# xiezheng-cs/PyTorch_Distributed_Template

Measured on AMD Instinct MI355X. Metric: images/sec (node) ResNet-18 DDP bs=1200/GPU at 1/2/4/8 MI355X, higher is better.
Workload: dtype bf16; 1 GPU; model=resnet18, global_batch=1200, parallelism=dp1, per_gpu_batch=1200, sync_bn=False, engine=native-hip, comm=none, grad_compress=none

## Files before the change

### csrc/bindings.cpp

```cpp
#include <torch/extension.h>
#include <ATen/hip/HIPContext.h>
#include <c10/hip/HIPCachingAllocator.h>
#include <c10/hip/HIPGuard.h>

#include <cstdio>
#include <algorithm>
#include <map>
#include <memory>
#include <mutex>
#include <optional>
#include <vector>
#include <stdexcept>
#include <string>

#include "common.h"
#include "dtypes.h"
#include "kernels/bn.h"
#include "kernels/bnact.h"
#include "kernels/conv1x1.h"
#include "kernels/conv_fwd.h"
#include "kernels/conv_l1.h"
#include "kernels/conv_wgrad.h"
#include "kernels/dwconv.h"
#include "kernels/fp32.h"
// ... 1446 lines not shown
  m.def("gconv_dgrad", &gconv_dgrad, py::arg("dy"), py::arg("wt"), py::arg("dx"), py::arg("N"), py::arg("P"),
        py::arg("Q"), py::arg("width"), py::arg("H"), py::arg("W"), py::arg("stride"), py::arg("phases"), py::arg("j"),
        py::arg("bm"), py::arg("bn"), py::arg("bn_y1") = py::none(), py::arg("bn_coef1") = py::none(),
        py::arg("bn_slots") = py::none());
  m.def("gconv_wgrad", &gconv_wgrad);
  m.def("gconv_slice", []() { return kGSlice; });
  m.def("gconv_wgrad_l1", &gconv_wgrad_l1);
  m.def("wgrad_reduce", &wgrad_reduce);
  m.def("wgrad_blocks_3x3c64", &wgrad_blocks_3x3c64);
  m.def("wgrad_3x3c64_supported", &wgrad_3x3c64_supported);
  m.def("conv_wgrad_3x3c64", &conv_wgrad_3x3c64, py::arg("x"), py::arg("dy"), py::arg("ws"), py::arg("N"), py::arg("H"),
        py::arg("W"), py::arg("pre_coef") = py::none());
  m.def("conv_fwd_pre", &conv_fwd_pre);
  m.def("conv1x1x", &conv1x1x);
  m.def("conv1x1x_supported", &conv1x1x_supported);
  m.def("conv_dgrad_persistent", &dgrad_persistent_kind);
  m.def("conv1x1x_mode", &conv1x1x_mode);
  m.def("conv1x1x_l1_mode", &conv1x1x_l1_mode);
  m.def("conv_fwd_pre_supported", &conv_fwd_pre_supported);
  m.def("bn_slot_sum", &bn_slot_sum);
  m.def("stat_slots", &stat_slots);
  m.def("conv_l1_set_pp", &pdt::conv_l1_set_pp, py::arg("mode"),
        "layer1 kernel choice: 1 = 8-wave ping-pong, 0 = 4-wave, -1 = PDT_CONV_L1_PP (default); returns the previous");
  m.def("conv32_set_halo", &pdt::conv32_set_halo, py::arg("on"),
        "fp32 3x3/s1 64-channel convolutions: 1 = halo kernel (default), 0 = per-tap "
        "restaging kernel; returns the previous setting");
  m.def("bn_finalize", &bn_finalize);
  m.def("bn_finalize_slots", &bn_finalize_slots);
  m.def("bn_bwd_finalize_slots", &bn_bwd_finalize_slots);
  m.def("bn_eval_coef", &bn_eval_coef);
  m.def("bn_apply", &bn_apply);
  m.def("bn_bwd_reduce_blocks", &bn_bwd_reduce_blocks);
  m.def("bn_bwd_reduce", &bn_bwd_reduce);
  m.def("bn_bwd_finalize", &bn_bwd_finalize);
  m.def("bn_bwd_apply", &bn_bwd_apply);
  m.def("bn_relu_maxpool", &bn_relu_maxpool, py::arg("y"), py::arg("coef"), py::arg("out"), py::arg("idx"),
        py::arg("N"), py::arg("H"), py::arg("W"), py::arg("C"), py::arg("pad") = 1);
  m.def("maxpool_bwd_relu", &maxpool_bwd_relu, py::arg("dp"), py::arg("idx"), py::arg("y"), py::arg("coef"),
        py::arg("dz"), py::arg("N"), py::arg("H"), py::arg("W"), py::arg("C"), py::arg("pad") = 1);
  m.def("stem_fwd", &stem_fwd);
  m.def("stem_fwd_supported", [](int64_t Hp, int64_t Wp, int64_t P, int64_t Q) {
    return pdt::stem_fwd_supported((int)Hp, (int)Wp, (int)P, (int)Q);
  });
  m.def("stem_pool_bwd_reduce", &stem_pool_bwd_reduce);
  m.def("stem_pool_bwd_reduce_out", &stem_pool_bwd_reduce_out);
  m.def("stem_pool_bwd_apply", &stem_pool_bwd_apply);
  m.def("bnact_stats", &bnact_stats, py::arg("x"), py::arg("slots"), py::arg("rows"), py::arg("C"));
// ... 66 lines not shown
```

### csrc/common.h

```cpp
#pragma once
#include <hip/hip_runtime.h>
#include <stdint.h>

#include "dtypes.h"

namespace pdt {

struct FastDiv {
  uint32_t mul;
  uint32_t shift;
};

inline FastDiv make_fastdiv(uint32_t d) {
  uint32_t s = 0;
  while ((2ull << s) <= d) ++s;
  if ((d & (d - 1)) == 0) return FastDiv{0u, s};
  const uint64_t m = ((1ull << (32 + s)) + d - 1) / d;
  return FastDiv{(uint32_t)m, s};
}

}

#ifdef __HIPCC__
#define PDT_DEVICE __device__ __forceinline__
// ... 113 lines not shown

PDT_DEVICE uint32_t fdiv(uint32_t x, FastDiv f) {
  return f.mul ? (__umulhi(x, f.mul) >> f.shift) : (x >> f.shift);
}

typedef __attribute__((address_space(3))) void lds_void_t;
constexpr uint32_t kOOB = 0x80000000u;

PDT_DEVICE __amdgpu_buffer_rsrc_t make_rsrc(const void* p, uint32_t bytes) {
  return __builtin_amdgcn_make_buffer_rsrc(const_cast<void*>(p), (short)0, (int)bytes, 0x00020000);
}

PDT_DEVICE void buf_lds16(__amdgpu_buffer_rsrc_t r, void* lds_dst, uint32_t voff) {
  __builtin_amdgcn_raw_ptr_buffer_load_lds(r, (lds_void_t*)lds_dst, 16, voff, 0, 0, 0);
}

PDT_DEVICE void buf_lds16_asm(__amdgpu_buffer_rsrc_t r, void* lds_dst, uint32_t voff) {
  const uint32_t m0v = (uint32_t)(uintptr_t)(lds_void_t*)lds_dst;
  asm volatile("s_mov_b32 m0, %0\n\tbuffer_load_dwordx4 %1, %2, 0 offen lds"
               :
               : "s"(m0v), "v"(voff), "s"(r)
               : "m0");
}

typedef uint32_t u32x4v __attribute__((ext_vector_type(4)));
typedef uint32_t u32x2v __attribute__((ext_vector_type(2)));
PDT_DEVICE u32x4v gload16_asm(const void* p) {
  u32x4v v;
  asm volatile("global_load_dwordx4 %0, %1, off" : "=v"(v) : "v"(p));
  return v;
}
PDT_DEVICE u32x2v gload8_asm(const void* p) {
  u32x2v v;
  asm volatile("global_load_dwordx2 %0, %1, off" : "=v"(v) : "v"(p));
  return v;
}

PDT_DEVICE int xcd_remap(int bid, int nwg) {
  const int q = nwg >> 3, r = nwg & 7;
  const int xcd = bid & 7, local = bid >> 3;
  return (xcd < r ? xcd * (q + 1) : r * (q + 1) + (xcd - r) * q) + local;
}

}
#endif

// ... 33 lines not shown
```

### csrc/kernels/conv_fwd.h

```cpp
#pragma once
#include <hip/hip_runtime.h>
#include <stdint.h>

#include "conv_geom.h"

namespace pdt {

constexpr int kStatSlots = 64;

void stat_rows_reduce_launch(const float* rows, int R, int CK, double* slots, hipStream_t s, int slots_ld = 0);


struct ConvFwdArgs : ConvGeom {
  const uint16_t* x;
  const uint16_t* w;
  uint16_t* y;
  const uint16_t* res;
  double* stats;
  int bnb;
  const uint16_t* bn_y1;
  const float* bn_coef1;
  const uint16_t* bn_y2;
  const float* bn_coef2;
  const uint8_t* bn_mask;
  int pair_skip;
  int res_phase = -1;
  int stage_out = 0;
  const float* pre_coef = nullptr;
  int ldy = 0, coef_ld = 0, stats_ld = 0;
  int nslice = 0;
  int64_t slice_wstride = 0;
  int srows_coff = 0;
};

void conv_fwd_launch(const ConvFwdArgs& a, int dtype, int bm, int bn, int bk, hipStream_t s);
int conv_fwd_m_tiles(int64_t M, int bm);

}
```

### csrc/kernels/conv_fwd.hip

```cpp
#include <cstdlib>

#include "../common.h"
#include "conv_fwd.h"
#include "conv_l1.h"

namespace pdt {

typedef __attribute__((address_space(3))) void lds_void;
typedef __attribute__((address_space(1))) void glb_void;

template <int CHUNKS>
PDT_DEVICE int swz(int row) { return (row >> 1) & (CHUNKS - 1); }

template <int DT, int EPI, int RES, int FN, int FM, int WN, int WM, int BN, int WAVES_M, int NW_, int SMEM = 0,
          bool PERM = false>
PDT_DEVICE void conv_epilogue(const ConvFwdArgs& a, f32x4_t (&acc)[FN][FM], int64_t m0, int n0, int tile_m, int wn,
                              int wm, int tid, int lane, char* smem) {
  using E = E16<DT>;
  const int fr = lane & 15, fq = lane >> 4;
  const int PQ = a.Pm * a.Qm;
  const FastDiv fd_pq{a.pq_mul, a.pq_shift}, fd_q{a.q_mul, a.q_shift};
  constexpr int KS = EPI == 0 ? 0 : (EPI == 4 ? 3 : 2);
  float sacc[FN][4][KS > 0 ? KS : 1];
#pragma unroll
  for (int i = 0; i < FN; ++i)
#pragma unroll
    for (int r = 0; r < 4; ++r)
#pragma unroll
      for (int k = 0; k < (KS > 0 ? KS : 1); ++k) sacc[i][r][k] = 0.f;

  constexpr int RED_BYTES = WAVES_M * BN * 3 * 4;
  float* cf = (float*)(smem + RED_BYTES);
  const int64_t LDY = a.ldy ? a.ldy : a.Kout;
  if constexpr (EPI >= 2) {
    const int CL = a.coef_ld ? a.coef_ld : a.Kout;
    for (int c = tid; c < BN; c += NW_ * 64) {
      const int n = n0 + c;
      cf[0 * BN + c] = a.bn_coef1[n];
      cf[1 * BN + c] = a.bn_coef1[CL + n];
      cf[2 * BN + c] = a.bn_coef1[2 * CL + n];
      cf[3 * BN + c] = a.bn_coef1[3 * CL + n];
      if constexpr (EPI == 4) {
        cf[4 * BN + c] = a.bn_coef2[2 * CL + n];
        cf[5 * BN + c] = a.bn_coef2[3 * CL + n];
      }
    }
    __syncthreads();
  }
  auto chan = [&](int i, int r) { return PERM ? (i >> 1) * 32 + 8 * fq + 4 * (i & 1) + r : i * 16 + 4 * fq + r; };
  static_assert(!PERM || FN % 2 == 0, "PERM pairs fragments");
  auto coef4 = [&](int q, int i) { return *(const float4*)(cf + q * BN + wn * WN + chan(i, 0)); };

  constexpr bool LY1 = EPI >= 2, LY2 = EPI == 4, LM = EPI == 3 || EPI == 4;
  static_assert(!LM || WN % 64 == 0, "bitmask epilogue needs 64-channel wave columns");
  constexpr int MW = LM ? WN / 64 : 1;
  constexpr int PER_J = FN * (2 * (RES != 0) + 2 * LY1 + 2 * LY2) + (LM ? 2 * MW : 0);
  constexpr int BUDGET = (FN * FM * 4 >= 128 ? 64 : 96) - (KS > 2 ? FN * 4 * (KS - 2) * 2 : 0);
  constexpr int JC = PER_J == 0 ? FM
                     : (8 * PER_J <= BUDGET && FM % 8 == 0) ? 8
                     : (4 * PER_J <= BUDGET && FM % 4 == 0) ? 4
                     : (2 * PER_J <= BUDGET && FM % 2 == 0) ? 2 : 1;
  static_assert(FM % JC == 0, "epilogue chunking");
  constexpr int BM_T = WAVES_M * WM;
  constexpr int SPITCH = BN * 2 + 16;
  constexpr int STG_OFF = 16384;
  constexpr bool FULL = SMEM >= STG_OFF + BM_T * SPITCH;
  constexpr bool PERGRP = !FULL && WAVES_M > 1 && EPI != 2 && SMEM >= STG_OFF + WM * SPITCH;
  constexpr bool CAN_STAGE = FULL || PERGRP;
  static_assert(!CAN_STAGE || RED_BYTES + 6 * BN * 4 <= STG_OFF, "epilogue LDS regions overlap");
  const bool stage = CAN_STAGE && a.stage_out;
  char* stg = smem + STG_OFF;
  const int srow0 = FULL ? wm * WM : 0;
  constexpr bool RC = RES == 2;
  const bool res_on = !RC || (int)blockIdx.y == a.res_phase;
  auto copy_rows = [&](int g) {
    constexpr int CPR = BN / 8;
    constexpr int SROWS = FULL ? BM_T : WM;
    for (int q = tid; q < SROWS * CPR; q += NW_ * 64) {
      const int row = q / CPR, ch = q - row * CPR;
      const int64_t m = m0 + (FULL ? 0 : g * WM) + row;
      if (m < a.M) {
        const int mm = (int)m;
        const int nimg = (int)fdiv((uint32_t)mm, fd_pq);
        const int rem = mm - nimg * PQ;
        const int i_ = (int)fdiv((uint32_t)rem, fd_q), j_ = rem - i_ * a.Qm;
        const int oh = i_ * a.ost_h + a.ooff_h, ow = j_ * a.ost_w + a.ooff_w;
        const int64_t ob = (((int64_t)nimg * a.OH + oh) * a.OW + ow) * LDY + n0 + ch * 8;
        *(uint4*)(a.y + ob) = *(const uint4*)(stg + row * SPITCH + ch * 16);
      }
    }
  };
  if constexpr (PERGRP) {
    if (stage)
      for (int g = 0; g < wm; ++g) {
        __syncthreads();
        copy_rows(g);
        __syncthreads();
      }
  }
#pragma unroll
  for (int jc = 0; jc < FM; jc += JC) {
    int64_t obase[JC];
    uint32_t rbase[RC ? JC : 1];
    bool valid[JC];
#pragma unroll
    for (int jj = 0; jj < JC; ++jj) {
      const int64_t m = m0 + wm * WM + (jc + jj) * 16 + fr;
      valid[jj] = m < a.M;
      const int mm = valid[jj] ? (int)m : 0;
      const int nimg = (int)fdiv((uint32_t)mm, fd_pq);
      const int rem = mm - nimg * PQ;
      const int i_ = (int)fdiv((uint32_t)rem, fd_q), j_ = rem - i_ * a.Qm;
      const int oh = i_ * a.ost_h + a.ooff_h, ow = j_ * a.ost_w + a.ooff_w;
      obase[jj] = (((int64_t)nimg * a.OH + oh) * a.OW + ow) * LDY;
      if constexpr (RC) rbase[jj] = (uint32_t)mm * (uint32_t)LDY;
    }
    uint2 p_res[RES ? JC : 1][RES ? FN : 1], p_y1[LY1 ? JC : 1][LY1 ? FN : 1], p_y2[LY2 ? JC : 1][LY2 ? FN : 1];
    uint64_t p_m[LM ? JC : 1][MW];
#pragma unroll
    for (int jj = 0; jj < JC; ++jj) {
      if constexpr (PERM) {
#pragma unroll
        for (int i = 0; i < FN; i += 2) {
          const int64_t o = obase[jj] + n0 + wn * WN + chan(i, 0);
          auto split = [&](uint2 (&dst)[FN], const uint4 v) {
            dst[i] = make_uint2(v.x, v.y);
            dst[i + 1] = make_uint2(v.z, v.w);
          };
          if constexpr (RES == 1) split(p_res[jj], *(const uint4*)(a.res + o));
          if constexpr (RC) split(p_res[jj], *(const uint4*)(a.res + rbase[jj] + (uint32_t)(n0 + wn * WN + chan(i, 0))));
          if constexpr (LY1) split(p_y1[jj], *(const uint4*)(a.bn_y1 + o));
          if constexpr (LY2) split(p_y2[jj], *(const uint4*)(a.bn_y2 + o));
        }
      } else {
#pragma unroll
        for (int i = 0; i < FN; ++i) {
          const int64_t o = obase[jj] + n0 + wn * WN + i * 16 + 4 * fq;
          if constexpr (RES == 1) p_res[jj][i] = *(const uint2*)(a.res + o);
          if constexpr (RC) p_res[jj][i] = *(const uint2*)(a.res + rbase[jj] + (uint32_t)(n0 + wn * WN + i * 16 + 4 * fq));
          if constexpr (LY1) p_y1[jj][i] = *(const uint2*)(a.bn_y1 + o);
          if constexpr (LY2) p_y2[jj][i] = *(const uint2*)(a.bn_y2 + o);
        }
      }
      if constexpr (LM) {
#pragma unroll
        for (int g = 0; g < MW; ++g)
          p_m[jj][g] = *(const uint64_t*)(a.bn_mask + ((obase[jj] + n0 + wn * WN + g * 64) >> 3));
      }
    }
#pragma unroll
    for (int jj = 0; jj < JC; ++jj) {
      if (!valid[jj]) continue;
      const int j = jc + jj;
      uint2 held = make_uint2(0u, 0u);
#pragma unroll
      for (int i = 0; i < FN; ++i) {
        const int n = n0 + wn * WN + chan(i, 0);
        const int64_t o = obase[jj] + n;
        float v[4] = {acc[i][j][0], acc[i][j][1], acc[i][j][2], acc[i][j][3]};
        if constexpr (RES) {
          uint2 rr = p_res[jj][i];
          if constexpr (RC) {
            rr.x = res_on ? rr.x : 0u;
            rr.y = res_on ? rr.y : 0u;
          }
          v[0] += E::to_f((uint16_t)(rr.x & 0xffff));
          v[1] += E::to_f((uint16_t)(rr.x >> 16));
          v[2] += E::to_f((uint16_t)(rr.y & 0xffff));
          v[3] += E::to_f((uint16_t)(rr.y >> 16));
        }
        float y1[4], y2[4];
        if constexpr (LY1) {
          const uint2 q1 = p_y1[jj][i];
          y1[0] = E::to_f((uint16_t)(q1.x & 0xffff)); y1[1] = E::to_f((uint16_t)(q1.x >> 16));
          y1[2] = E::to_f((uint16_t)(q1.y & 0xffff)); y1[3] = E::to_f((uint16_t)(q1.y >> 16));
          if constexpr (EPI == 2) {
            const float4 sc = coef4(0, i), sh = coef4(1, i);
            if (!(y1[0] * sc.x + sh.x > 0.f)) v[0] = 0.f;
            if (!(y1[1] * sc.y + sh.y > 0.f)) v[1] = 0.f;
            if (!(y1[2] * sc.z + sh.z > 0.f)) v[2] = 0.f;
            if (!(y1[3] * sc.w + sh.w > 0.f)) v[3] = 0.f;
          } else {
            const uint32_t mb = (uint32_t)(p_m[jj][chan(i, 0) >> 6] >> (chan(i, 0) & 63));
            if (!(mb & 1u)) v[0] = 0.f;
            if (!(mb & 2u)) v[1] = 0.f;
            if (!(mb & 4u)) v[2] = 0.f;
            if (!(mb & 8u)) v[3] = 0.f;
          }
        }
        if constexpr (LY2) {
          const uint2 q2 = p_y2[jj][i];
          y2[0] = E::to_f((uint16_t)(q2.x & 0xffff)); y2[1] = E::to_f((uint16_t)(q2.x >> 16));
          y2[2] = E::to_f((uint16_t)(q2.y & 0xffff)); y2[3] = E::to_f((uint16_t)(q2.y >> 16));
        }
        uint2 packed;
        packed.x = E::pack2(v[0], v[1]);
        packed.y = E::pack2(v[2], v[3]);
        const uint16_t ov[4] = {(uint16_t)packed.x, (uint16_t)(packed.x >> 16), (uint16_t)packed.y,
                                (uint16_t)(packed.y >> 16)};
        if (CAN_STAGE && stage) {
          if constexpr (PERM) {
            if (i & 1)
              *(uint4*)(stg + (srow0 + j * 16 + fr) * SPITCH + (wn * WN + chan(i, 0) - 4) * 2) =
                  make_uint4(held.x, held.y, packed.x, packed.y);
            else
              held = packed;
          } else {
            *(uint2*)(stg + (srow0 + j * 16 + fr) * SPITCH + (wn * WN + chan(i, 0)) * 2) = packed;
          }
        } else if constexpr (PERM) {
          if (i & 1)
            *(uint4*)(a.y + o - 4) = make_uint4(held.x, held.y, packed.x, packed.y);
          else
            held = packed;
        } else {
          *(uint2*)(a.y + o) = packed;
        }
        if constexpr (EPI == 1) {
#pragma unroll
          for (int r = 0; r < 4; ++r) {
            const float q = E::to_f(ov[r]);
            sacc[i][r][0] += q;
            sacc[i][r][1] += q * q;
          }
        } else if constexpr (EPI >= 2) {
          const float4 mu = coef4(2, i), is = coef4(3, i);
          const float m1[4] = {mu.x, mu.y, mu.z, mu.w}, i1[4] = {is.x, is.y, is.z, is.w};
#pragma unroll
          for (int r = 0; r < 4; ++r) {
            const float dz = E::to_f(ov[r]);
            sacc[i][r][0] += dz;
            sacc[i][r][1] += dz * (y1[r] - m1[r]) * i1[r];
          }
          if constexpr (EPI == 4) {
            const float4 mu2 = coef4(4, i), is2 = coef4(5, i);
            const float m2[4] = {mu2.x, mu2.y, mu2.z, mu2.w}, i2[4] = {is2.x, is2.y, is2.z, is2.w};
#pragma unroll
            for (int r = 0; r < 4; ++r) sacc[i][r][2] += E::to_f(ov[r]) * (y2[r] - m2[r]) * i2[r];
          }
        }
      }
    }
  }

  if constexpr (CAN_STAGE) {
    if (stage) {
      if constexpr (PERGRP) {
        for (int g = wm; g < WAVES_M; ++g) {
          __syncthreads();
          copy_rows(g);
          __syncthreads();
        }
      } else {
        __syncthreads();
        copy_rows(0);
      }
    }
  }

  if constexpr (KS > 0) {
    constexpr int KO = EPI == 4 ? 4 : 2;
#pragma unroll
    for (int i = 0; i < FN; ++i)
#pragma unroll
      for (int r = 0; r < 4; ++r)
#pragma unroll
        for (int k = 0; k < KS; ++k) sacc[i][r][k] = row16_sum(sacc[i][r][k]);
    float* red = (float*)smem;
    __syncthreads();
    if (fr == 15) {
#pragma unroll
      for (int i = 0; i < FN; ++i)
#pragma unroll
        for (int r = 0; r < 4; ++r) {
          const int nl = wn * WN + chan(i, r);
#pragma unroll
          for (int k = 0; k < KS; ++k) red[(wm * BN + nl) * KS + k] = sacc[i][r][k];
        }
// ... 9 lines not shown
        for (int k = 0; k < KS; ++k) t[k] += red[(w * BN + tid) * KS + k];
      const int64_t row = (a.nphase > 0 ? (int64_t)blockIdx.y * a.srows_pp : 0) + tile_m;
      const int64_t sld = a.nslice > 1 ? (int64_t)a.nslice * a.Kout : a.Kout;
      float* dst = a.srows + (row * sld + a.srows_coff + n0 + tid) * KO;
      if constexpr (EPI == 4)
        *(float4*)dst = make_float4(t[0], t[1], t[0], t[2]);
      else
        *(float2*)dst = make_float2(t[0], t[1]);
    }
  }
}

template <int EPI, int BN_>
PDT_DEVICE void zero_stat_row(const ConvFwdArgs& a, int nthreads) {
  if constexpr (EPI != 0) {
    constexpr int KO = EPI == 4 ? 4 : 2;
    const int tm = (int)blockIdx.x / a.n_tiles, tn = (int)blockIdx.x - tm * a.n_tiles;
    const int64_t sld = a.nslice > 1 ? (int64_t)a.nslice * a.Kout : a.Kout;
    float* dst = a.srows + (((int64_t)blockIdx.y * a.srows_pp + tm) * sld + a.srows_coff) * KO + (int64_t)tn * BN_ * KO;
    for (int i = threadIdx.x; i < BN_ * KO; i += nthreads) dst[i] = 0.f;
  }
}

template <int DT, int BM, int BN, int BK, int WAVES_N, int EPI, int RES, int STAGES, int NW>
__global__ __launch_bounds__(NW * 64, (STAGES * (BN + BM) * BK * 2 <= 81920 || NW == 8) ? 2 : 1)
void conv_fwd_kernel(ConvFwdArgs args) {
  ConvFwdArgs a = args;
  const uint16_t* wbase = args.w;
  if (args.nslice > 1) {
    const int sl = blockIdx.z;
    a.x += (int64_t)sl * a.Kout;
    a.y += (int64_t)sl * a.Kout;
    wbase += (int64_t)sl * args.slice_wstride;
    a.w = wbase;
    if (a.bn_y1 != nullptr) a.bn_y1 += (int64_t)sl * a.Kout;
    if (a.bn_coef1 != nullptr) a.bn_coef1 += sl * a.Kout;
    a.srows_coff = sl * a.Kout;
  }
  if (args.nphase > 0 && !select_phase(a, args, wbase, blockIdx.y)) {
    zero_stat_row<EPI, BN>(a, NW * 64);
    return;
  }
  using E = E16<DT>;
  typedef typename E::vec8 vec8;
  constexpr int WAVES_M = NW / WAVES_N;
  constexpr int WN = BN / WAVES_N;
  constexpr int WM = BM / WAVES_M;
// ... 146 lines not shown
        asm volatile("s_waitcnt vmcnt(0)" ::: "memory");
    };
    static_assert(S <= 4, "wait_ahead covers at most two stages in flight");
    if (ksteps > 0) {
#pragma unroll
      for (int p = 0; p < S - 1; ++p)
        if (p < ksteps) stage_load(p);
      int buf = 0;
      for (int ks = 0; ks < ksteps; ++ks) {
        const int ahead = min(S - 2, ksteps - 1 - ks);
        wait_ahead(ahead);
        __builtin_amdgcn_s_barrier();
        if (ks + S - 1 < ksteps) stage_load(buf == 0 ? S - 1 : buf - 1);
        __builtin_amdgcn_s_setprio(1);
        compute_stage(smem + buf * STAGE);
        __builtin_amdgcn_s_setprio(0);
        buf = buf == S - 1 ? 0 : buf + 1;
      }
      asm volatile("s_waitcnt lgkmcnt(0)" ::: "memory");
      __builtin_amdgcn_s_barrier();
    }
  }

  conv_epilogue<DT, EPI, RES, FN, FM, WN, WM, BN, WAVES_M, NW, STAGES * STAGE, PERM>(a, acc, m0, n0, tile_m, wn, wm, tid,
                                                                             lane, smem);
}

template <int N>
PDT_DEVICE void vm_wait() {
  static_assert(N >= 0 && N < 64, "vmcnt range");
  __builtin_amdgcn_s_waitcnt((N & 0xF) | ((N >> 4) << 14) | (0x7 << 4) | (0xF << 8));
}

template <int DT, int BM, int BN, int EPI, int RES, bool PP_STAGE = (EPI != 2)>
__global__ __launch_bounds__(512) void conv_pp_kernel(ConvFwdArgs args) {
  ConvFwdArgs a = args;
  if (args.nphase > 0 && !select_phase(a, args, args.w, blockIdx.y)) {
    zero_stat_row<EPI, BN>(a, 512);
    return;
  }
  using E = E16<DT>;
  typedef typename E::vec8 vec8;
  constexpr int NW = 8, WN = 64, WM = 128;
  constexpr int WAVES_N = BN / WN, WAVES_M = NW / WAVES_N;
  static_assert(WAVES_N * WAVES_M == NW && WAVES_M * WM == BM, "pp tile geometry");
  constexpr int FN = 4, FM = 8;
  constexpr int ROWB = 128;
  constexpr int XH = (BM / 2) * ROWB;
  constexpr int WH = (BN / 2) * ROWB;
  constexpr int NX = XH / 1024 / NW;
  constexpr int NWI = WH / 1024 / NW;
  static_assert(NX * 1024 * NW == XH && NWI * 1024 * NW == WH, "pp DMA split");
  constexpr int BUF = 2 * XH + 2 * WH;
  constexpr int OX0 = 0, OX1 = XH, OW0 = 2 * XH, OW1 = 2 * XH + WH;
  __shared__ __attribute__((aligned(1024))) char smem[2 * BUF];

  const int tid = threadIdx.x;
  const int lane = tid & 63;
  const int wave = __builtin_amdgcn_readfirstlane(tid >> 6);
  const int grp = wave >> 2;
  const int wn = wave % WAVES_N, wm = wave / WAVES_N;

  const int nwg = a.m_tiles * a.n_tiles;
  const int bid = xcd_remap(blockIdx.x, nwg);
  const int tile_m = bid / a.n_tiles, tile_n = bid % a.n_tiles;
  const int64_t m0 = (int64_t)tile_m * BM;
  const int n0 = tile_n * BN;

  const int PQ = a.Pm * a.Qm;
  const FastDiv fd_pq{a.pq_mul, a.pq_shift}, fd_q{a.q_mul, a.q_shift};
  const int TU = a.T * a.U;
  const int csteps = a.C >> 6;
  const int ksteps = TU * csteps;

  const __amdgpu_buffer_rsrc_t rx = make_rsrc(a.x, (uint32_t)a.N * a.H * a.W * a.cs * 2u);
  const __amdgpu_buffer_rsrc_t rw = make_rsrc(a.w, (uint32_t)a.Kout * TU * a.C * 2u);

  const int lrow = lane >> 3, pchunk = lane & 7;
// ... 114 lines not shown
    for (int ks = 0; ks < ksteps; ++ks) {
      const char* cb = smem + (ks & 1) * BUF;
      char* nb = smem + ((ks + 1) & 1) * BUF;
      const bool more = ks + 1 < ksteps;
      if (more) advance();
      if (more) { dma_x(nb, 0); vm_wait<2 * NX>(); } else { vm_wait<NX>(); }
      read_x(cb + OX0);
      read_w(w0r, cb + OW0);
      compute(w0r, 0, 0);
      if (more) { dma_w(nb, 0); vm_wait<NX + NWI>(); } else { vm_wait<0>(); }
      read_w(w1r, cb + OW1);
      compute(w1r, 0, 1);
      if (more) dma_w(nb, 1);
      read_x(cb + OX1);
      compute(w1r, 1, 1);
      if (more) { dma_x(nb, 1); vm_wait<NWI + NX>(); }
      compute(w0r, 1, 0);
    }
    if (grp == 0) __builtin_amdgcn_s_barrier();
    asm volatile("s_waitcnt vmcnt(0) lgkmcnt(0)" ::: "memory");
    __builtin_amdgcn_s_barrier();
  }

  conv_epilogue<DT, EPI, RES, FN, FM, WN, WM, BN, WAVES_M, NW, PP_STAGE ? 2 * BUF : 0, true>(a, acc, m0, n0, tile_m, wn,
                                                                                        wm, tid, lane, smem);
}

template <int DT, int BM, int BN>
static void launch_pp(const ConvFwdArgs& args, int gx, hipStream_t s) {
  ConvFwdArgs a = args;
  a.stage_out = 0;
  if (a.nslice > 1)
    pdt_hip_fail("conv_pp: slice-batched (grouped) launches run on the generic kernel", hipErrorInvalidValue, __FILE__,
                 __LINE__);
  dim3 grid(gx, a.nphase > 0 ? a.nphase : 1), block(512);
  const int rs = a.res == nullptr ? 0 : (a.res_phase >= 0 && a.nphase > 0 ? 2 : 1);
  const int epi = a.bnb ? a.bnb + 1 : (a.stats != nullptr ? 1 : 0);
#define PDT_K(E_, R_) hipLaunchKernelGGL((conv_pp_kernel<DT, BM, BN, E_, R_>), grid, block, 0, s, a)
  if (epi == 0) {
    if (rs == 1) PDT_K(0, 1); else if (rs == 2) PDT_K(0, 2); else PDT_K(0, 0);
  } else if (epi == 1 && rs != 2) {
    if (rs) PDT_K(1, 1); else PDT_K(1, 0);
  } else if (epi == 2 && !rs) {
    PDT_K(2, 0);
  } else if (epi == 3 && rs) {
    if (rs == 2) PDT_K(3, 2); else PDT_K(3, 1);
  } else if (epi == 4 && rs) {
    if (rs == 2) PDT_K(4, 2); else PDT_K(4, 1);
  } else {
    pdt_hip_fail("conv_pp: unsupported epilogue variant", hipErrorInvalidValue, __FILE__, __LINE__);
  }
#undef PDT_K
}

template <int DT, int BM, int BN, int BK, int WAVES_N, int STAGES, int NW>
static void launch_cfg(const ConvFwdArgs& a, int gx, hipStream_t s) {
  dim3 grid(gx, a.nphase > 0 ? a.nphase : 1, a.nslice > 1 ? a.nslice : 1), block(NW * 64);
  const int rs = a.res == nullptr ? 0 : (a.res_phase >= 0 && a.nphase > 0 ? 2 : 1);
  const int epi = a.bnb ? a.bnb + 1 : (a.stats != nullptr ? 1 : 0);
#define PDT_K(E_, R_) hipLaunchKernelGGL((conv_fwd_kernel<DT, BM, BN, BK, WAVES_N, E_, R_, STAGES, NW>), grid, block, 0, s, a)
  if (epi == 0) {
    if (rs == 1) PDT_K(0, 1); else if (rs == 2) PDT_K(0, 2); else PDT_K(0, 0);
  } else if (epi == 1 && rs != 2) {
    if (rs) PDT_K(1, 1); else PDT_K(1, 0);
  } else if constexpr ((((BK == 64 && STAGES == 2) || (BK == 32 && STAGES == 3)) && (BN == 128 || BN == 64) &&
                        (BM * BN == 4096 * NW || (BM == 256 && BN == 128 && NW == 4))) ||
                       (BM == 256 && BN == 256)) {
    if (epi == 2 && !rs) PDT_K(2, 0);
    else if (epi == 3 && rs) { if (rs == 2) PDT_K(3, 2); else PDT_K(3, 1); }
    else if (epi == 4 && rs) { if (rs == 2) PDT_K(4, 2); else PDT_K(4, 1); }
    else pdt_hip_fail("conv_fwd: unsupported BN-backward epilogue variant", hipErrorInvalidValue, __FILE__, __LINE__);
  } else {
    pdt_hip_fail("conv_fwd: BN-backward epilogue needs a 128x128 or 256x64 tile", hipErrorInvalidValue,
                 __FILE__, __LINE__);
  }
#undef PDT_K
}

template <int DT>
static void launch_tile(const ConvFwdArgs& a, int gx, int bm, int bn, int bk, hipStream_t s);

template <int DT>
static void launch_dt(ConvFwdArgs a, int bm, int bn, int bk, hipStream_t s) {
  a.stage_out = 0;
  int gx = 0;
  const int srows = conv_geom_plan(a, bm, bn, &gx);
  if (gx == 0) return;
  const int KO = a.bnb == 3 ? 4 : 2;
  const int nsl = a.nslice > 1 ? a.nslice : 1;
  Scratch part(a.stats ? (size_t)srows * a.Kout * nsl * KO * sizeof(float) : 0, s);
  a.srows = part.as<float>();
  launch_tile<DT>(a, gx, bm, bn, bk, s);
  if (a.stats) stat_rows_reduce_launch(a.srows, srows, a.Kout * nsl * KO, a.stats, s, a.stats_ld);
}

template <int DT>
static void launch_tile(const ConvFwdArgs& a, int gx, int bm, int bn, int bk, hipStream_t s) {
#define PDT_CFGN(BM_, BN_, BK_, WN_, ST_, NW_)            \
  if (bm == BM_ && bn == BN_ && bk == BK_) {               \
    launch_cfg<DT, BM_, BN_, BK_, WN_, ST_, NW_>(a, gx, s); \
    return;                                                \
  }
#define PDT_CFG(BM_, BN_, BK_, WN_, ST_) PDT_CFGN(BM_, BN_, BK_, WN_, ST_, 4)
  {
    const bool dg = a.nphase > 0;
    const bool pp = bk == 64 && a.C % 64 == 0 && ((bm == 256 && bn == 256) || (bm == 512 && bn == 128));
    if (pp && dg)
// ... 89 lines not shown
```

Baseline: 62390 images/s.

## Stream BN-backward epilogue operands through a per-wave LDS ring via buffer-to-LDS loads

Adds a RING variant of the conv epilogue for the BN-backward dgrad cases (EPI 3/4 with residual). It prefetches the residual, y1, y2 and mask operands for several output chunks into a per-wave LDS ring using buffer_load...lds, and waits on those loads with explicit vmcnt values, so global loads overlap the epilogue math instead of stalling on register-held chunks. It also removes the unused stage_out path that staged output through LDS. The ring is on by default and can be toggled with an env var or a new binding. In exchange it enlarges LDS in the pp kernel and relies on hand-tuned waitcnt counts.

Measured after the change: 62960 images/s, median of 6. Within noise of the previous version (+0.9%).

```diff
diff --git a/csrc/bindings.cpp b/csrc/bindings.cpp
--- a/csrc/bindings.cpp
+++ b/csrc/bindings.cpp
@@ -1492,7 +1492,10 @@
   m.def("stat_slots", &stat_slots);
   m.def("conv_l1_set_pp", &pdt::conv_l1_set_pp, py::arg("mode"),
         "layer1 kernel choice: 1 = 8-wave ping-pong, 0 = 4-wave, -1 = PDT_CONV_L1_PP (default); returns the previous");
-  m.def("conv32_set_halo", &pdt::conv32_set_halo, py::arg("on"),
+  m.def("conv_set_epi_ring", &pdt::conv_set_epi_ring, py::arg("mode"),
+        "operand ring of the block-output BN-backward dgrad epilogues: 1 = on, 0 = register chunks, "
+        "-1 = PDT_EPI_RING (default: on); returns the previous");
+  m.def("conv32_set_halo",&pdt::conv32_set_halo, py::arg("on"),
         "fp32 3x3/s1 64-channel convolutions: 1 = halo kernel (default), 0 = per-tap "
         "restaging kernel; returns the previous setting");
   m.def("bn_finalize", &bn_finalize);
diff --git a/csrc/common.h b/csrc/common.h
--- a/csrc/common.h
+++ b/csrc/common.h
@@ -159,6 +159,16 @@
                : "s"(m0v), "v"(voff), "s"(r)
                : "m0");
 }
+PDT_DEVICE void buf_lds4_lo32_asm(__amdgpu_buffer_rsrc_t r, void* lds_dst, uint32_t voff) {
+  const uint32_t m0v = (uint32_t)(uintptr_t)(lds_void_t*)lds_dst;
+  uint32_t hi;
+  asm volatile(
+      "s_mov_b32 m0, %1\n\ts_mov_b32 %0, exec_hi\n\ts_mov_b32 exec_hi, 0\n\t"
+      "buffer_load_dword %2, %3, 0 offen lds\n\ts_mov_b32 exec_hi, %0"
+      : "=&s"(hi)
+      : "s"(m0v), "v"(voff), "s"(r)
+      : "m0");
+}
 
 typedef uint32_t u32x4v __attribute__((ext_vector_type(4)));
 typedef uint32_t u32x2v __attribute__((ext_vector_type(2)));
diff --git a/csrc/kernels/conv_fwd.h b/csrc/kernels/conv_fwd.h
--- a/csrc/kernels/conv_fwd.h
+++ b/csrc/kernels/conv_fwd.h
@@ -25,7 +25,6 @@
   const uint8_t* bn_mask;
   int pair_skip;
   int res_phase = -1;
-  int stage_out = 0;
   const float* pre_coef = nullptr;
   int ldy = 0, coef_ld = 0, stats_ld = 0;
   int nslice = 0;
@@ -35,5 +34,6 @@
 
 void conv_fwd_launch(const ConvFwdArgs& a, int dtype, int bm, int bn, int bk, hipStream_t s);
 int conv_fwd_m_tiles(int64_t M, int bm);
+int conv_set_epi_ring(int mode);
 
 }
diff --git a/csrc/kernels/conv_fwd.hip b/csrc/kernels/conv_fwd.hip
--- a/csrc/kernels/conv_fwd.hip
+++ b/csrc/kernels/conv_fwd.hip
@@ -1,4 +1,6 @@
 #include <cstdlib>
+#include <type_traits>
+#include <utility>
 
 #include "../common.h"
 #include "conv_fwd.h"
@@ -12,8 +14,23 @@
 template <int CHUNKS>
 PDT_DEVICE int swz(int row) { return (row >> 1) & (CHUNKS - 1); }
 
+template <class F, int... Is>
+PDT_DEVICE void static_for_impl(F&& f, std::integer_sequence<int, Is...>) {
+  (f(std::integral_constant<int, Is>{}), ...);
+}
+template <int N, class F>
+PDT_DEVICE void static_for(F&& f) {
+  static_for_impl(f, std::make_integer_sequence<int, N>{});
+}
+
+template <int N>
+PDT_DEVICE void epi_vm_wait() {
+  static_assert(N >= 0 && N < 64, "vmcnt range");
+  asm volatile("s_waitcnt vmcnt(%0)" ::"n"(N) : "memory");
+}
+
 template <int DT, int EPI, int RES, int FN, int FM, int WN, int WM, int BN, int WAVES_M, int NW_, int SMEM = 0,
-          bool PERM = false>
+          bool PERM = false, bool RING = false>
 PDT_DEVICE void conv_epilogue(const ConvFwdArgs& a, f32x4_t (&acc)[FN][FM], int64_t m0, int n0, int tile_m, int wn,
                               int wm, int tid, int lane, char* smem) {
   using E = E16<DT>;
@@ -32,7 +49,7 @@
   constexpr int RED_BYTES = WAVES_M * BN * 3 * 4;
   float* cf = (float*)(smem + RED_BYTES);
   const int64_t LDY = a.ldy ? a.ldy : a.Kout;
-  if constexpr (EPI >= 2) {
+  auto stage_coefs = [&]() __attribute__((always_inline)) {
     const int CL = a.coef_ld ? a.coef_ld : a.Kout;
     for (int c = tid; c < BN; c += NW_ * 64) {
       const int n = n0 + c;
@@ -46,7 +63,8 @@
       }
     }
     __syncthreads();
-  }
+  };
+  if constexpr (EPI >= 2 && !RING) stage_coefs();
   auto chan = [&](int i, int r) { return PERM ? (i >> 1) * 32 + 8 * fq + 4 * (i & 1) + r : i * 16 + 4 * fq + r; };
   static_assert(!PERM || FN % 2 == 0, "PERM pairs fragments");
   auto coef4 = [&](int q, int i) { return *(const float4*)(cf + q * BN + wn * WN + chan(i, 0)); };
@@ -61,199 +79,236 @@
                      : (4 * PER_J <= BUDGET && FM % 4 == 0) ? 4
                      : (2 * PER_J <= BUDGET && FM % 2 == 0) ? 2 : 1;
   static_assert(FM % JC == 0, "epilogue chunking");
-  constexpr int BM_T = WAVES_M * WM;
-  constexpr int SPITCH = BN * 2 + 16;
-  constexpr int STG_OFF = 16384;
-  constexpr bool FULL = SMEM >= STG_OFF + BM_T * SPITCH;
-  constexpr bool PERGRP = !FULL && WAVES_M > 1 && EPI != 2 && SMEM >= STG_OFF + WM * SPITCH;
-  constexpr bool CAN_STAGE = FULL || PERGRP;
-  static_assert(!CAN_STAGE || RED_BYTES + 6 * BN * 4 <= STG_OFF, "epilogue LDS regions overlap");
-  const bool stage = CAN_STAGE && a.stage_out;
-  char* stg = smem + STG_OFF;
-  const int srow0 = FULL ? wm * WM : 0;
   constexpr bool RC = RES == 2;
   const bool res_on = !RC || (int)blockIdx.y == a.res_phase;
-  auto copy_rows = [&](int g) {
-    constexpr int CPR = BN / 8;
-    constexpr int SROWS = FULL ? BM_T : WM;
-    for (int q = tid; q < SROWS * CPR; q += NW_ * 64) {
-      const int row = q / CPR, ch = q - row * CPR;
-      const int64_t m = m0 + (FULL ? 0 : g * WM) + row;
-      if (m < a.M) {
-        const int mm = (int)m;
-        const int nimg = (int)fdiv((uint32_t)mm, fd_pq);
-        const int rem = mm - nimg * PQ;
-        const int i_ = (int)fdiv((uint32_t)rem, fd_q), j_ = rem - i_ * a.Qm;
-        const int oh = i_ * a.ost_h + a.ooff_h, ow = j_ * a.ost_w + a.ooff_w;
-        const int64_t ob = (((int64_t)nimg * a.OH + oh) * a.OW + ow) * LDY + n0 + ch * 8;
-        *(uint4*)(a.y + ob) = *(const uint4*)(stg + row * SPITCH + ch * 16);
-      }
-    }
-  };
-  if constexpr (PERGRP) {
-    if (stage)
-      for (int g = 0; g < wm; ++g) {
-        __syncthreads();
-        copy_rows(g);
-        __syncthreads();
-      }
-  }
-#pragma unroll
-  for (int jc = 0; jc < FM; jc += JC) {
-    int64_t obase[JC];
-    uint32_t rbase[RC ? JC : 1];
-    bool valid[JC];
-#pragma unroll
-    for (int jj = 0; jj < JC; ++jj) {
-      const int64_t m = m0 + wm * WM + (jc + jj) * 16 + fr;
-      valid[jj] = m < a.M;
-      const int mm = valid[jj] ? (int)m : 0;
-      const int nimg = (int)fdiv((uint32_t)mm, fd_pq);
-      const int rem = mm - nimg * PQ;
-      const int i_ = (int)fdiv((uint32_t)rem, fd_q), j_ = rem - i_ * a.Qm;
-      const int oh = i_ * a.ost_h + a.ooff_h, ow = j_ * a.ost_w + a.ooff_w;
-      obase[jj] = (((int64_t)nimg * a.OH + oh) * a.OW + ow) * LDY;
-      if constexpr (RC) rbase[jj] = (uint32_t)mm * (uint32_t)LDY;
-    }
-    uint2 p_res[RES ? JC : 1][RES ? FN : 1], p_y1[LY1 ? JC : 1][LY1 ? FN : 1], p_y2[LY2 ? JC : 1][LY2 ? FN : 1];
-    uint64_t p_m[LM ? JC : 1][MW];
-#pragma unroll
-    for (int jj = 0; jj < JC; ++jj) {
+  auto pixel = [&](int j, bool& ok, int64_t& ob, uint32_t& rb) __attribute__((always_inline)) {
+    const int64_t m = m0 + wm * WM + j * 16 + fr;
+    ok = m < a.M;
+    const int mm = ok ? (int)m : 0;
+    const int nimg = (int)fdiv((uint32_t)mm, fd_pq);
+    const int rem = mm - nimg * PQ;
+    const int i_ = (int)fdiv((uint32_t)rem, fd_q), j_ = rem - i_ * a.Qm;
+    const int oh = i_ * a.ost_h + a.ooff_h, ow = j_ * a.ost_w + a.ooff_w;
+    ob = (((int64_t)nimg * a.OH + oh) * a.OW + ow) * LDY;
+    rb = (uint32_t)mm * (uint32_t)LDY;
+  };
+  auto emit = [&](int j, int64_t ob, const uint2 (&pr)[RES ? FN : 1], const uint2 (&py1)[LY1 ? FN : 1],
+                  const uint2 (&py2)[LY2 ? FN : 1], const uint64_t (&pm)[MW]) __attribute__((always_inline)) {
+    uint2 held = make_uint2(0u, 0u);
+#pragma unroll
+    for (int i = 0; i < FN; ++i) {
+      const int n = n0 + wn * WN + chan(i, 0);
+      const int64_t o = ob + n;
+      float v[4] = {acc[i][j][0], acc[i][j][1], acc[i][j][2], acc[i][j][3]};
+      if constexpr (RES) {
+        uint2 rr = pr[i];
+        if constexpr (RC) {
+          rr.x = res_on ? rr.x : 0u;
+          rr.y = res_on ? rr.y : 0u;
+        }
+        v[0] += E::to_f((uint16_t)(rr.x & 0xffff));
+        v[1] += E::to_f((uint16_t)(rr.x >> 16));
+        v[2] += E::to_f((uint16_t)(rr.y & 0xffff));
+        v[3] += E::to_f((uint16_t)(rr.y >> 16));
+      }
+      float y1[4], y2[4];
+      if constexpr (LY1) {
+        const uint2 q1 = py1[i];
+        y1[0] = E::to_f((uint16_t)(q1.x & 0xffff)); y1[1] = E::to_f((uint16_t)(q1.x >> 16));
+        y1[2] = E::to_f((uint16_t)(q1.y & 0xffff)); y1[3] = E::to_f((uint16_t)(q1.y >> 16));
+        if constexpr (EPI == 2) {
+          const float4 sc = coef4(0, i), sh = coef4(1, i);
+          if (!(y1[0] * sc.x + sh.x > 0.f)) v[0] = 0.f;
+          if (!(y1[1] * sc.y + sh.y > 0.f)) v[1] = 0.f;
+          if (!(y1[2] * sc.z + sh.z > 0.f)) v[2] = 0.f;
+          if (!(y1[3] * sc.w + sh.w > 0.f)) v[3] = 0.f;
+        } else {
+          const uint32_t mb = (uint32_t)(pm[chan(i, 0) >> 6] >> (chan(i, 0) & 63));
+          if (!(mb & 1u)) v[0] = 0.f;
+          if (!(mb & 2u)) v[1] = 0.f;
+          if (!(mb & 4u)) v[2] = 0.f;
+          if (!(mb & 8u)) v[3] = 0.f;
+        }
+      }
+      if constexpr (LY2) {
+        const uint2 q2 = py2[i];
+        y2[0] = E::to_f((uint16_t)(q2.x & 0xffff)); y2[1] = E::to_f((uint16_t)(q2.x >> 16));
+        y2[2] = E::to_f((uint16_t)(q2.y & 0xffff)); y2[3] = E::to_f((uint16_t)(q2.y >> 16));
+      }
+      uint2 packed;
+      packed.x = E::pack2(v[0], v[1]);
+      packed.y = E::pack2(v[2], v[3]);
+      const uint16_t ov[4] = {(uint16_t)packed.x, (uint16_t)(packed.x >> 16), (uint16_t)packed.y,
+                              (uint16_t)(packed.y >> 16)};
       if constexpr (PERM) {
-#pragma unroll
-        for (int i = 0; i < FN; i += 2) {
-          const int64_t o = obase[jj] + n0 + wn * WN + chan(i, 0);
-          auto split = [&](uint2 (&dst)[FN], const uint4 v) {
-            dst[i] = make_uint2(v.x, v.y);
-            dst[i + 1] = make_uint2(v.z, v.w);
+        if (i & 1)
+          *(uint4*)(a.y + o - 4) = make_uint4(held.x, held.y, packed.x, packed.y);
+        else
+          held = packed;
+      } else {
+        *(uint2*)(a.y + o) = packed;
+      }
+      if constexpr (EPI == 1) {
+#pragma unroll
+        for (int r = 0; r < 4; ++r) {
+          const float q = E::to_f(ov[r]);
+          sacc[i][r][0] += q;
+          sacc[i][r][1] += q * q;
+        }
+      } else if constexpr (EPI >= 2) {
+        const float4 mu = coef4(2, i), is = coef4(3, i);
+        const float m1[4] = {mu.x, mu.y, mu.z, mu.w}, i1[4] = {is.x, is.y, is.z, is.w};
+#pragma unroll
+        for (int r = 0; r < 4; ++r) {
+          const float dz = E::to_f(ov[r]);
+          sacc[i][r][0] += dz;
+          sacc[i][r][1] += dz * (y1[r] - m1[r]) * i1[r];
+        }
+        if constexpr (EPI == 4) {
+          const float4 mu2 = coef4(4, i), is2 = coef4(5, i);
+          const float m2[4] = {mu2.x, mu2.y, mu2.z, mu2.w}, i2[4] = {is2.x, is2.y, is2.z, is2.w};
+#pragma unroll
+          for (int r = 0; r < 4; ++r) sacc[i][r][2] += E::to_f(ov[r]) * (y2[r] - m2[r]) * i2[r];
+        }
+      }
+      if constexpr (RING) {
+#pragma unroll
+        for (int r = 0; r < 4; ++r)
+#pragma unroll
+          for (int k = 0; k < KS; ++k) asm volatile("" : "+v"(sacc[i][r][k]));
+      }
+    }
+  };
+
+  if constexpr (RING) {
+    static_assert(PERM && LM && MW == 1 && RES != 0 && JC < FM, "operand ring: EPI 3 / 4 on the 128 x 64 wave tile");
+    constexpr int NP = FN / 2;
+    constexpr int NT = 2 + LY2;
+    constexpr int ND = NT * NP + 1;
+    constexpr int NS = NP;
+    constexpr int CHUNK_B = NT * NP * 1024, MSLOT_B = 128, MASK_OFF = 12288, RING_OFF = 16384;
+    constexpr int DFIT = (SMEM - RING_OFF) / (NW_ * CHUNK_B);
+    constexpr int DMAX = NW_ == 8 ? 3 : 2;
+    constexpr int D = DFIT < DMAX ? DFIT : DMAX;
+    static_assert(D >= 2 && D <= FM, "operand ring: at least two chunks in flight");
+    static_assert(RED_BYTES + 6 * BN * 4 <= MASK_OFF && MASK_OFF + NW_ * D * MSLOT_B <= RING_OFF,
+                  "epilogue LDS regions overlap");
+    const int wave = wm * (BN / WN) + wn;
+    char* ring = smem + RING_OFF + wave * (D * CHUNK_B);
+    char* mring = smem + MASK_OFF + wave * (D * MSLOT_B);
+    const uint32_t ybytes = (uint32_t)a.N * (uint32_t)a.OH * (uint32_t)a.OW * (uint32_t)LDY * 2u;
+    const __amdgpu_buffer_rsrc_t r_res = make_rsrc(a.res, RC ? (uint32_t)a.M * (uint32_t)LDY * 2u : ybytes);
+    const __amdgpu_buffer_rsrc_t r_y1 = make_rsrc(a.bn_y1, ybytes);
+    const __amdgpu_buffer_rsrc_t r_y2 = make_rsrc(LY2 ? a.bn_y2 : a.bn_y1, ybytes);
+    const __amdgpu_buffer_rsrc_t r_m = make_rsrc(a.bn_mask, ybytes >> 4);
+    const uint32_t ncol = (uint32_t)(n0 + wn * WN);
+    const int64_t mrow = m0 + wm * WM + fr;
+    uint32_t eo[FM];
+    auto run = [&](auto tail_c) __attribute__((always_inline)) {
+      constexpr bool TAIL = decltype(tail_c)::value;
+      auto issue = [&](int j) __attribute__((always_inline)) {
+        bool ok;
+        int64_t ob;
+        uint32_t rb;
+        pixel(j, ok, ob, rb);
+        if constexpr (!TAIL) ok = true;
+        eo[j] = (uint32_t)ob + ncol;
+        char* slot = ring + (j % D) * CHUNK_B;
+#pragma unroll
+        for (int p = 0; p < NP; ++p) {
+          const uint32_t c = (uint32_t)chan(2 * p, 0);
+          const uint32_t vo = ok ? (eo[j] + c) * 2u : kOOB;
+          if constexpr (RC)
+            buf_lds16_asm(r_res, slot + p * 1024,
+                          ok && res_on ? (rb + ncol + c) * 2u : kOOB);
+          else
+            buf_lds16_asm(r_res, slot + p * 1024, vo);
+          buf_lds16_asm(r_y1, slot + (NP + p) * 1024, vo);
+          if constexpr (LY2) buf_lds16_asm(r_y2, slot + (2 * NP + p) * 1024, vo);
+        }
+        buf_lds4_lo32_asm(r_m, mring + (j % D) * MSLOT_B, ok ? (eo[j] >> 3) + (uint32_t)fq * 4u : kOOB);
+      };
+#pragma unroll
+      for (int j = 0; j < D; ++j) issue(j);
+      stage_coefs();
+      static_for<FM>([&](auto j_c) __attribute__((always_inline)) {
+        constexpr int j = decltype(j_c)::value;
+        constexpr int behind = (j + D - 1 < FM - 1 ? j + D - 1 : FM - 1) - j;
+        constexpr int nst = j < D ? j : D;
+        constexpr int slot_i = j % D;
+        epi_vm_wait<TAIL ? 0 : behind * ND + nst * NS>();
+        const char* slot = ring + slot_i * CHUNK_B + lane * 16;
+        uint2 p_res[FN], p_y1[FN], p_y2[LY2 ? FN : 1];
+        uint64_t p_m[1];
+#pragma unroll
+        for (int p = 0; p < NP; ++p) {
+          auto split = [&](uint2* dst, const uint4 v) {
+            dst[2 * p] = make_uint2(v.x, v.y);
+            dst[2 * p + 1] = make_uint2(v.z, v.w);
           };
-          if constexpr (RES == 1) split(p_res[jj], *(const uint4*)(a.res + o));
-          if constexpr (RC) split(p_res[jj], *(const uint4*)(a.res + rbase[jj] + (uint32_t)(n0 + wn * WN + chan(i, 0))));
-          if constexpr (LY1) split(p_y1[jj], *(const uint4*)(a.bn_y1 + o));
-          if constexpr (LY2) split(p_y2[jj], *(const uint4*)(a.bn_y2 + o));
-        }
-      } else {
-#pragma unroll
-        for (int i = 0; i < FN; ++i) {
-          const int64_t o = obase[jj] + n0 + wn * WN + i * 16 + 4 * fq;
-          if constexpr (RES == 1) p_res[jj][i] = *(const uint2*)(a.res + o);
-          if constexpr (RC) p_res[jj][i] = *(const uint2*)(a.res + rbase[jj] + (uint32_t)(n0 + wn * WN + i * 16 + 4 * fq));
-          if constexpr (LY1) p_y1[jj][i] = *(const uint2*)(a.bn_y1 + o);
-          if constexpr (LY2) p_y2[jj][i] = *(const uint2*)(a.bn_y2 + o);
-        }
-      }
-      if constexpr (LM) {
-#pragma unroll
-        for (int g = 0; g < MW; ++g)
-          p_m[jj][g] = *(const uint64_t*)(a.bn_mask + ((obase[jj] + n0 + wn * WN + g * 64) >> 3));
-      }
-    }
-#pragma unroll
-    for (int jj = 0; jj < JC; ++jj) {
-      if (!valid[jj]) continue;
-      const int j = jc + jj;
-      uint2 held = make_uint2(0u, 0u);
-#pragma unroll
-      for (int i = 0; i < FN; ++i) {
-        const int n = n0 + wn * WN + chan(i, 0);
-        const int64_t o = obase[jj] + n;
-        float v[4] = {acc[i][j][0], acc[i][j][1], acc[i][j][2], acc[i][j][3]};
-        if constexpr (RES) {
-          uint2 rr = p_res[jj][i];
-          if constexpr (RC) {
-            rr.x = res_on ? rr.x : 0u;
-            rr.y = res_on ? rr.y : 0u;
+          split(p_res, *(const uint4*)(slot + p * 1024));
+          split(p_y1, *(const uint4*)(slot + (NP + p) * 1024));
+          if constexpr (LY2) split(p_y2, *(const uint4*)(slot + (2 * NP + p) * 1024));
+        }
+        {
+          const uint32_t* mw = (const uint32_t*)(mring + slot_i * MSLOT_B) + fr;
+          p_m[0] = (uint64_t)mw[0] | ((uint64_t)mw[16] << 32);
+        }
+        asm volatile("s_waitcnt lgkmcnt(0)" ::: "memory");
+        if constexpr (j + D < FM) issue(j + D);
+        if (TAIL && !(mrow + j * 16 < a.M)) return;
+        emit(j, (int64_t)(eo[j] - ncol), p_res, p_y1, p_y2, p_m);
+      });
+    };
+    if (m0 + WAVES_M * WM > a.M)
+      run(std::true_type{});
+    else
+      run(std::false_type{});
+  } else {
+#pragma unroll
+    for (int jc = 0; jc < FM; jc += JC) {
+      int64_t obase[JC];
+      uint32_t rbase[JC];
+      bool valid[JC];
+#pragma unroll
+      for (int jj = 0; jj < JC; ++jj) pixel(jc + jj, valid[jj], obase[jj], rbase[jj]);
+      uint2 p_res[JC][RES ? FN : 1], p_y1[JC][LY1 ? FN : 1], p_y2[JC][LY2 ? FN : 1];
+      uint64_t p_m[JC][MW];
+#pragma unroll
+      for (int jj = 0; jj < JC; ++jj) {
+        if constexpr (PERM) {
+#pragma unroll
+          for (int i = 0; i < FN; i += 2) {
+            const int64_t o = obase[jj] + n0 + wn * WN + chan(i, 0);
+            auto split = [&](uint2* dst, const uint4 v) {
+              dst[i] = make_uint2(v.x, v.y);
+              dst[i + 1] = make_uint2(v.z, v.w);
+            };
+            if constexpr (RES == 1) split(p_res[jj], *(const uint4*)(a.res + o));
+            if constexpr (RC) split(p_res[jj], *(const uint4*)(a.res + rbase[jj] + (uint32_t)(n0 + wn * WN + chan(i, 0))));
+            if constexpr (LY1) split(p_y1[jj], *(const uint4*)(a.bn_y1 + o));
+            if constexpr (LY2) split(p_y2[jj], *(const uint4*)(a.bn_y2 + o));
           }
-          v[0] += E::to_f((uint16_t)(rr.x & 0xffff));
-          v[1] += E::to_f((uint16_t)(rr.x >> 16));
-          v[2] += E::to_f((uint16_t)(rr.y & 0xffff));
-          v[3] += E::to_f((uint16_t)(rr.y >> 16));
-        }
-        float y1[4], y2[4];
-        if constexpr (LY1) {
-          const uint2 q1 = p_y1[jj][i];
-          y1[0] = E::to_f((uint16_t)(q1.x & 0xffff)); y1[1] = E::to_f((uint16_t)(q1.x >> 16));
-          y1[2] = E::to_f((uint16_t)(q1.y & 0xffff)); y1[3] = E::to_f((uint16_t)(q1.y >> 16));
-          if constexpr (EPI == 2) {
-            const float4 sc = coef4(0, i), sh = coef4(1, i);
-            if (!(y1[0] * sc.x + sh.x > 0.f)) v[0] = 0.f;
-            if (!(y1[1] * sc.y + sh.y > 0.f)) v[1] = 0.f;
-            if (!(y1[2] * sc.z + sh.z > 0.f)) v[2] = 0.f;
-            if (!(y1[3] * sc.w + sh.w > 0.f)) v[3] = 0.f;
-          } else {
-            const uint32_t mb = (uint32_t)(p_m[jj][chan(i, 0) >> 6] >> (chan(i, 0) & 63));
-            if (!(mb & 1u)) v[0] = 0.f;
-            if (!(mb & 2u)) v[1] = 0.f;
-            if (!(mb & 4u)) v[2] = 0.f;
-            if (!(mb & 8u)) v[3] = 0.f;
+        } else {
+#pragma unroll
+          for (int i = 0; i < FN; ++i) {
+            const int64_t o = obase[jj] + n0 + wn * WN + i * 16 + 4 * fq;
+            if constexpr (RES == 1) p_res[jj][i] = *(const uint2*)(a.res + o);
+            if constexpr (RC) p_res[jj][i] = *(const uint2*)(a.res + rbase[jj] + (uint32_t)(n0 + wn * WN + i * 16 + 4 * fq));
+            if constexpr (LY1) p_y1[jj][i] = *(const uint2*)(a.bn_y1 + o);
+            if constexpr (LY2) p_y2[jj][i] = *(const uint2*)(a.bn_y2 + o);
           }
         }
-        if constexpr (LY2) {
-          const uint2 q2 = p_y2[jj][i];
-          y2[0] = E::to_f((uint16_t)(q2.x & 0xffff)); y2[1] = E::to_f((uint16_t)(q2.x >> 16));
-          y2[2] = E::to_f((uint16_t)(q2.y & 0xffff)); y2[3] = E::to_f((uint16_t)(q2.y >> 16));
-        }
-        uint2 packed;
-        packed.x = E::pack2(v[0], v[1]);
-        packed.y = E::pack2(v[2], v[3]);
-        const uint16_t ov[4] = {(uint16_t)packed.x, (uint16_t)(packed.x >> 16), (uint16_t)packed.y,
-                                (uint16_t)(packed.y >> 16)};
-        if (CAN_STAGE && stage) {
-          if constexpr (PERM) {
-            if (i & 1)
-              *(uint4*)(stg + (srow0 + j * 16 + fr) * SPITCH + (wn * WN + chan(i, 0) - 4) * 2) =
-                  make_uint4(held.x, held.y, packed.x, packed.y);
-            else
-              held = packed;
-          } else {
-            *(uint2*)(stg + (srow0 + j * 16 + fr) * SPITCH + (wn * WN + chan(i, 0)) * 2) = packed;
-          }
-        } else if constexpr (PERM) {
-          if (i & 1)
-            *(uint4*)(a.y + o - 4) = make_uint4(held.x, held.y, packed.x, packed.y);
-          else
-            held = packed;
-        } else {
-          *(uint2*)(a.y + o) = packed;
-        }
-        if constexpr (EPI == 1) {
-#pragma unroll
-          for (int r = 0; r < 4; ++r) {
-            const float q = E::to_f(ov[r]);
-            sacc[i][r][0] += q;
-            sacc[i][r][1] += q * q;
-          }
-        } else if constexpr (EPI >= 2) {
-          const float4 mu = coef4(2, i), is = coef4(3, i);
-          const float m1[4] = {mu.x, mu.y, mu.z, mu.w}, i1[4] = {is.x, is.y, is.z, is.w};
-#pragma unroll
-          for (int r = 0; r < 4; ++r) {
-            const float dz = E::to_f(ov[r]);
-            sacc[i][r][0] += dz;
-            sacc[i][r][1] += dz * (y1[r] - m1[r]) * i1[r];
-          }
-          if constexpr (EPI == 4) {
-            const float4 mu2 = coef4(4, i), is2 = coef4(5, i);
-            const float m2[4] = {mu2.x, mu2.y, mu2.z, mu2.w}, i2[4] = {is2.x, is2.y, is2.z, is2.w};
-#pragma unroll
-            for (int r = 0; r < 4; ++r) sacc[i][r][2] += E::to_f(ov[r]) * (y2[r] - m2[r]) * i2[r];
-          }
-        }
-      }
-    }
-  }
-
-  if constexpr (CAN_STAGE) {
-    if (stage) {
-      if constexpr (PERGRP) {
-        for (int g = wm; g < WAVES_M; ++g) {
-          __syncthreads();
-          copy_rows(g);
-          __syncthreads();
-        }
-      } else {
-        __syncthreads();
-        copy_rows(0);
+        if constexpr (LM) {
+#pragma unroll
+          for (int g = 0; g < MW; ++g)
+            p_m[jj][g] = *(const uint64_t*)(a.bn_mask + ((obase[jj] + n0 + wn * WN + g * 64) >> 3));
+        }
+      }
+#pragma unroll
+      for (int jj = 0; jj < JC; ++jj) {
+        if (!valid[jj]) continue;
+        emit(jc + jj, obase[jj], p_res[jj], p_y1[jj], p_y2[jj], p_m[jj]);
       }
     }
   }
@@ -309,7 +364,7 @@
   }
 }
 
-template <int DT, int BM, int BN, int BK, int WAVES_N, int EPI, int RES, int STAGES, int NW>
+template <int DT, int BM, int BN, int BK, int WAVES_N, int EPI, int RES, int STAGES, int NW, bool RING = false>
 __global__ __launch_bounds__(NW * 64, (STAGES * (BN + BM) * BK * 2 <= 81920 || NW == 8) ? 2 : 1)
 void conv_fwd_kernel(ConvFwdArgs args) {
   ConvFwdArgs a = args;
@@ -502,8 +557,8 @@
     }
   }
 
-  conv_epilogue<DT, EPI, RES, FN, FM, WN, WM, BN, WAVES_M, NW, STAGES * STAGE, PERM>(a, acc, m0, n0, tile_m, wn, wm, tid,
-                                                                             lane, smem);
+  conv_epilogue<DT, EPI, RES, FN, FM, WN, WM, BN, WAVES_M, NW, STAGES * STAGE, PERM, RING>(a, acc, m0, n0, tile_m, wn, wm,
+                                                                                   tid, lane, smem);
 }
 
 template <int N>
@@ -512,7 +567,7 @@
   __builtin_amdgcn_s_waitcnt((N & 0xF) | ((N >> 4) << 14) | (0x7 << 4) | (0xF << 8));
 }
 
-template <int DT, int BM, int BN, int EPI, int RES, bool PP_STAGE = (EPI != 2)>
+template <int DT, int BM, int BN, int EPI, int RES, bool RING = false>
 __global__ __launch_bounds__(512) void conv_pp_kernel(ConvFwdArgs args) {
   ConvFwdArgs a = args;
   if (args.nphase > 0 && !select_phase(a, args, args.w, blockIdx.y)) {
@@ -533,7 +588,10 @@
   static_assert(NX * 1024 * NW == XH && NWI * 1024 * NW == WH, "pp DMA split");
   constexpr int BUF = 2 * XH + 2 * WH;
   constexpr int OX0 = 0, OX1 = XH, OW0 = 2 * XH, OW1 = 2 * XH + WH;
-  __shared__ __attribute__((aligned(1024))) char smem[2 * BUF];
+  constexpr int RING_B = RING ? 16384 + NW * 3 * (EPI == 4 ? 3 : 2) * 2048 : 0;
+  constexpr int SMEM_B = RING_B > 2 * BUF ? RING_B : 2 * BUF;
+  static_assert(SMEM_B <= 163840, "LDS");
+  __shared__ __attribute__((aligned(1024))) char smem[SMEM_B];
 
   const int tid = threadIdx.x;
   const int lane = tid & 63;
@@ -694,14 +752,28 @@
     __builtin_amdgcn_s_barrier();
   }
 
-  conv_epilogue<DT, EPI, RES, FN, FM, WN, WM, BN, WAVES_M, NW, PP_STAGE ? 2 * BUF : 0, true>(a, acc, m0, n0, tile_m, wn,
-                                                                                        wm, tid, lane, smem);
+  conv_epilogue<DT, EPI, RES, FN, FM, WN, WM, BN, WAVES_M, NW, SMEM_B, true, RING>(a, acc, m0, n0, tile_m, wn, wm, tid,
+                                                                            lane, smem);
+}
+
+static int g_epi_ring = -1;
+static bool epi_ring_on(const ConvFwdArgs& a) {
+  static const bool ring_env = [] {
+    const char* e = getenv("PDT_EPI_RING");
+    return !(e && e[0] == '0');
+  }();
+  const int64_t ybytes = (int64_t)a.N * a.OH * a.OW * (a.ldy ? a.ldy : a.Kout) * 2;
+  return (g_epi_ring >= 0 ? g_epi_ring != 0 : ring_env) && ybytes < ((int64_t)1 << 31);
+}
+
+int conv_set_epi_ring(int mode) {
+  const int old = g_epi_ring;
+  g_epi_ring = mode;
+  return old;
 }
 
 template <int DT, int BM, int BN>
-static void launch_pp(const ConvFwdArgs& args, int gx, hipStream_t s) {
-  ConvFwdArgs a = args;
-  a.stage_out = 0;
+static void launch_pp(const ConvFwdArgs& a, int gx, hipStream_t s) {
   if (a.nslice > 1)
     pdt_hip_fail("conv_pp: slice-batched (grouped) launches run on the generic kernel", hipErrorInvalidValue, __FILE__,
                  __LINE__);
@@ -715,10 +787,18 @@
     if (rs) PDT_K(1, 1); else PDT_K(1, 0);
   } else if (epi == 2 && !rs) {
     PDT_K(2, 0);
-  } else if (epi == 3 && rs) {
-    if (rs == 2) PDT_K(3, 2); else PDT_K(3, 1);
-  } else if (epi == 4 && rs) {
-    if (rs == 2) PDT_K(4, 2); else PDT_K(4, 1);
+  } else if ((epi == 3 || epi == 4) && rs) {
+#define PDT_KR(E_, R_) hipLaunchKernelGGL((conv_pp_kernel<DT, BM, BN, E_, R_, true>), grid, block, 0, s, a)
+    const bool ring = epi_ring_on(a);
+    if (ring) PDT_COUNT("conv_epi_ring");
+    if (epi == 3) {
+      if (ring) { if (rs == 2) PDT_KR(3, 2); else PDT_KR(3, 1); }
+      else { if (rs == 2) PDT_K(3, 2); else PDT_K(3, 1); }
+    } else {
+      if (ring) { if (rs == 2) PDT_KR(4, 2); else PDT_KR(4, 1); }
+      else { if (rs == 2) PDT_K(4, 2); else PDT_K(4, 1); }
+    }
+#undef PDT_KR
   } else {
     pdt_hip_fail("conv_pp: unsupported epilogue variant", hipErrorInvalidValue, __FILE__, __LINE__);
   }
@@ -738,6 +818,17 @@
   } else if constexpr ((((BK == 64 && STAGES == 2) || (BK == 32 && STAGES == 3)) && (BN == 128 || BN == 64) &&
                         (BM * BN == 4096 * NW || (BM == 256 && BN == 128 && NW == 4))) ||
                        (BM == 256 && BN == 256)) {
+    if constexpr (BM == 256 && BN == 128 && NW == 4 && STAGES == 3) {
+      if ((epi == 3 || epi == 4) && rs && a.nslice <= 1 && epi_ring_on(a)) {
+#define PDT_KR(E_, R_) \
+  hipLaunchKernelGGL((conv_fwd_kernel<DT, BM, BN, BK, WAVES_N, E_, R_, STAGES, NW, true>), grid, block, 0, s, a)
+        PDT_COUNT("conv_epi_ring");
+        if (epi == 3) { if (rs == 2) PDT_KR(3, 2); else PDT_KR(3, 1); }
+        else { if (rs == 2) PDT_KR(4, 2); else PDT_KR(4, 1); }
+#undef PDT_KR
+        return;
+      }
+    }
     if (epi == 2 && !rs) PDT_K(2, 0);
     else if (epi == 3 && rs) { if (rs == 2) PDT_K(3, 2); else PDT_K(3, 1); }
     else if (epi == 4 && rs) { if (rs == 2) PDT_K(4, 2); else PDT_K(4, 1); }
@@ -754,7 +845,6 @@
 
 template <int DT>
 static void launch_dt(ConvFwdArgs a, int bm, int bn, int bk, hipStream_t s) {
-  a.stage_out = 0;
   int gx = 0;
   const int srows = conv_geom_plan(a, bm, bn, &gx);
   if (gx == 0) return;
```
